# hyunlord/hnm_recommendation

Measured on AMD Instinct MI355X. Metric: recommendations/sec (batched users, K=12) at 1/2/4/8 MI355X; % HBM roofline, higher is better.
Workload: dtype f16+f32; 1 GPU; ncf: BASELINE configs[1] NeuralCF dim=64, full H&M shape, batch=4096 users/rank, K=12; users=1371980, items=105542, batch_per_rank=4096, k=12, parallelism=single, model=NeuralCF, mf_dim=64, weights=init, scan=certified f16 pre-filter + exact fp32 re-scoring (ncf_cert.hip)

## Files before the change

hnm_recommendation_amd/_lib.py:

```python
from __future__ import annotations

import ctypes as C
import os
import threading
import weakref

import torch

PKG = os.path.dirname(os.path.abspath(__file__))
LIB_PATH = os.environ.get("HNM_LIB_PATH") or os.path.join(PKG, "libhnm_mi355x.so")

HNM_OK, HNM_EINVAL, HNM_EOOB, HNM_EHIP, HNM_ENOMEM, HNM_EUNSUPPORTED, HNM_ECOLL = 0, -1, -2, -3, -4, -5, -6

_p = C.c_void_p
_i64 = C.c_int64
_i32 = C.c_int32
_f32 = C.c_float


class NcfWeights(C.Structure):
    _fields_ = [("gmf_user", _p), ("gmf_item", _p), ("mlp_user", _p), ("mlp_item", _p),
                ("w1", _p), ("b1", _p), ("w2", _p), ("b2", _p), ("wp", _p), ("bp", _p),
                ("num_users", _i64), ("num_items", _i64), ("mf", _i32), ("h0", _i32),
                ("h1", _i32), ("h2", _i32), ("item_proj", _p)]
# ... 258 lines not shown
    check(fn("hnm_ctx_enable_timing")(ctx(device), int(on)), "hnm_ctx_enable_timing")


def kernel_timing(device):
    t = C.c_double()
    n = _i64()
    check(fn("hnm_ctx_timing")(ctx(device), C.byref(t), C.byref(n)), "hnm_ctx_timing")
    return t.value, n.value


HNM_OPT_PREFILTER = 1
HNM_OPT_STATS = 3
HNM_OPT_STRIDED = 4
HNM_OPT_DEEP_MFMA = 5
HNM_OPT_LINEAR_MFMA = 6


def set_option(device, option, value):
    idx = _dev_index(device)
    ctx(device)
    with _lock:
        _opts.setdefault(idx, {})[int(option)] = int(value)
    for c in _device_ctxs(idx):
        check(fn("hnm_ctx_set_option")(c.handle, int(option), int(value)), "hnm_ctx_set_option")


def set_prefilter(device, on=True):
    set_option(device, HNM_OPT_PREFILTER, int(bool(on)))


# ... 16 lines not shown
```

hnm_recommendation_amd/csrc/api.hip:

```cpp
#include <stdlib.h>
#include <string.h>

#include "hnm_device.h"
#include "hnm_internal.h"

static thread_local char g_err[512] = "";

void hnm_set_error(const char* fmt, ...) {
  va_list ap;
  va_start(ap, fmt);
  vsnprintf(g_err, sizeof(g_err), fmt, ap);
  va_end(ap);
}

extern "C" int hnm_abi_version(void) { return HNM_ABI_VERSION; }
extern "C" const char* hnm_last_error(void) { return g_err; }

extern "C" hnm_status hnm_ctx_create(int device, hnm_ctx** out) {
  HNM_REQUIRE(out, HNM_EINVAL, "hnm_ctx_create: out is NULL");
  int ndev = 0;
  HNM_HIP_CHECK(hipGetDeviceCount(&ndev));
  HNM_REQUIRE(device >= 0 && device < ndev, HNM_EINVAL, "hnm_ctx_create: no device %d (%d visible)",
              device, ndev);
  const HnmDeviceGuard guard(device);
  hnm_ctx* c = (hnm_ctx*)calloc(1, sizeof(hnm_ctx));
  HNM_REQUIRE(c, HNM_ENOMEM, "hnm_ctx_create: out of host memory");
  c->device = device;
  c->stream = 0;
  hipDeviceProp_t prop;
  if (hipGetDeviceProperties(&prop, device) == hipSuccess) c->num_cus = prop.multiProcessorCount;
  if (c->num_cus <= 0) c->num_cus = 256;
  c->prefilter = 1;
  c->strided = 0;
  c->deep_mfma = 1;
#ifndef HNM_LINEAR_MFMA_DEFAULT
#define HNM_LINEAR_MFMA_DEFAULT 1
#endif
  c->linear_mfma = HNM_LINEAR_MFMA_DEFAULT;
  if (hipMalloc((void**)&c->err_dev, 64) != hipSuccess) {
    free(c);
    hnm_set_error("hnm_ctx_create: hipMalloc of the error word failed");
    return HNM_ENOMEM;
  }
  HNM_HIP_CHECK(hipMemset(c->err_dev, 0, 64));
  HNM_HIP_CHECK(hipEventCreateWithFlags(&c->chain_ev, hipEventDisableTiming));
  HNM_HIP_CHECK(hipStreamCreateWithFlags(&c->side, hipStreamNonBlocking));
  HNM_HIP_CHECK(hipEventCreateWithFlags(&c->side_in, hipEventDisableTiming));
  HNM_HIP_CHECK(hipEventCreateWithFlags(&c->side_out, hipEventDisableTiming));
  c->stats_dev = reinterpret_cast<unsigned long long*>(reinterpret_cast<char*>(c->err_dev) + 8);
  *out = c;
  return HNM_OK;
}

// ... 43 lines not shown
    case HNM_OPT_PREFILTER:
      ctx->prefilter = value != 0;
      return HNM_OK;
    case HNM_OPT_STATS:
      ctx->stats_on = value != 0;
      return HNM_OK;
    case HNM_OPT_STRIDED:
      ctx->strided = value != 0;
      return HNM_OK;
    case HNM_OPT_DEEP_MFMA:
      ctx->deep_mfma = value != 0;
      return HNM_OK;
    case HNM_OPT_LINEAR_MFMA:
      ctx->linear_mfma = value != 0;
      return HNM_OK;
    default:
      hnm_set_error("hnm_ctx_set_option: unknown option %d", option);
      return HNM_EINVAL;
  }
}

extern "C" hnm_status hnm_ctx_prefilter_stats(hnm_ctx* ctx, int64_t* out, int reset) {
  HNM_CTX_DEVICE(ctx);
  return hnm_ctx_prefilter_stats_ex(ctx, out, 3, reset);
}

extern "C" hnm_status hnm_ctx_prefilter_stats_ex(hnm_ctx* ctx, int64_t* out, int n, int reset) {
  HNM_CTX_DEVICE(ctx);
  HNM_REQUIRE(ctx && out, HNM_EINVAL, "ctx/out is NULL");
  HNM_REQUIRE(n >= 1 && n <= HNM_STATS_N, HNM_EINVAL, "prefilter_stats: 1 <= n <= %d", HNM_STATS_N);
// ... 164 lines not shown
extern "C" hnm_status hnm_gather_rows_f32(hnm_ctx* ctx, const float* table, int64_t rows,
                                          int64_t ld, int d, const int64_t* ids, int64_t n,
                                          float* out, int64_t ldo) {
  HNM_CTX_DEVICE(ctx);
  HNM_REQUIRE(ctx && table && ((ids && out) || n == 0), HNM_EINVAL, "gather: NULL argument");
  HNM_REQUIRE(d > 0 && ld >= d && ldo >= d && rows > 0, HNM_EINVAL, "gather: bad shape");
  if (n <= 0) return HNM_OK;
  const bool vec4 = (d % 4 == 0) && (ld % 4 == 0) && (ldo % 4 == 0) &&
                    ((uintptr_t)table % 16 == 0) && ((uintptr_t)out % 16 == 0);
  hipLaunchKernelGGL(gather_rows_kernel, dim3((unsigned)hnm_cdiv(n, 4)), dim3(256), 0,
                     ctx->stream, table, rows, ld, d, ids, n, out, ldo, ctx->err_dev, vec4);
  HNM_LAUNCH_CHECK();
  return HNM_OK;
}

#define LIN_TN 64
#define LIN_TK 32
template <int LIN_TM, bool VEC>
__global__ __launch_bounds__(256) void linear_rows_kernel(
    const float* __restrict__ X, int64_t ldx, const int64_t* __restrict__ ids, int64_t x_rows,
    int64_t M, int K, const float* __restrict__ W, int64_t ldw, const float* __restrict__ bias,
    int N, float* __restrict__ Y, int64_t ldy, int pair_permute, unsigned* err) {
  constexpr int RPT = LIN_TM / 16;
  constexpr int XP = LIN_TM + (VEC ? 4 : 1), WP = LIN_TN + (VEC ? 4 : 1);
  __shared__ __attribute__((aligned(16))) float xs[LIN_TK][XP];
  __shared__ __attribute__((aligned(16))) float ws[LIN_TK][WP];
  const int t = threadIdx.x;
  const int64_t m0 = (int64_t)blockIdx.x * LIN_TM;
  const int n0 = blockIdx.y * LIN_TN;
  const int tr = (t >> 4) * RPT;
  const int tc = (t & 15) * 4;
  float acc[RPT][4] = {};
// ... 84 lines not shown
    for (int j = 0; j < 4; ++j) {
      const int n = n0 + tc + j;
      if (n >= N) continue;
      float v = acc[i][j];
      if (bias) v += bias[n];
      const int64_t c = pair_permute ? (int64_t)(n & 1) * (ldy / 2) + (n >> 1) : n;
      Y[m * ldy + c] = v;
    }
  }
}

__global__ __launch_bounds__(256) void linear_rows_mfma_kernel(
    const float* __restrict__ X, int64_t ldx, const int64_t* __restrict__ ids, int64_t x_rows,
    int64_t M, int K, const float* __restrict__ W, int64_t ldw, const float* __restrict__ bias,
    int N, float* __restrict__ Y, int64_t ldy, int pair_permute, unsigned* err) {
  constexpr int RS = LIN_TK + 1;
  __shared__ float xs[64 * RS];
  __shared__ float ws[64 * RS];
  const int t = threadIdx.x, lane = t & 63, wave = t >> 6;
  const int i = lane & 31, h = lane >> 5;
  const int64_t m0 = (int64_t)blockIdx.x * 64;
  const int n0 = blockIdx.y * LIN_TN;
  const int wr = 32 * (wave >> 1), wc = 32 * (wave & 1);
  f32x16 acc = {};
  for (int k0 = 0; k0 < K; k0 += LIN_TK) {
    for (int e = t; e < 64 * LIN_TK / 4; e += 256) {
      const int rr = e / (LIN_TK / 4), kq = 4 * (e % (LIN_TK / 4));
      const int64_t m = m0 + rr;
      float4 v = make_float4(0.f, 0.f, 0.f, 0.f);
      if (m < M) {
        const int64_t src = ids ? ids[m] : m;
        if (src < 0 || src >= x_rows) {
          if (kq == 0) hnm_flag(err, HNM_ERR_OOB);
          v = make_float4(__builtin_nanf(""), __builtin_nanf(""), __builtin_nanf(""),
                          __builtin_nanf(""));
        } else {
          v = *reinterpret_cast<const float4*>(X + src * ldx + k0 + kq);
        }
      }
      float* xr = xs + rr * RS + kq;
      xr[0] = v.x; xr[1] = v.y; xr[2] = v.z; xr[3] = v.w;
    }
    for (int e = t; e < LIN_TN * LIN_TK / 4; e += 256) {
      const int nn = e / (LIN_TK / 4), kq = 4 * (e % (LIN_TK / 4));
      float4 v = make_float4(0.f, 0.f, 0.f, 0.f);
      if (n0 + nn < N) v = *reinterpret_cast<const float4*>(W + (int64_t)(n0 + nn) * ldw + k0 + kq);
      float* wr4 = ws + nn * RS + kq;
      wr4[0] = v.x; wr4[1] = v.y; wr4[2] = v.z; wr4[3] = v.w;
    }
    __syncthreads();
    const float* xa = xs + (wr + i) * RS + h;
    const float* wb = ws + (wc + i) * RS + h;
#pragma unroll
    for (int st = 0; st < LIN_TK / 2; ++st) acc = mfma32x32x2(xa[2 * st], wb[2 * st], acc);
    __syncthreads();
  }
  const int n = n0 + wc + i;
  if (n >= N) return;
  const float bn = bias ? bias[n] : 0.f;
  const int64_t c = pair_permute ? (int64_t)(n & 1) * (ldy / 2) + (n >> 1) : n;
#pragma unroll
  for (int r = 0; r < 16; ++r) {
    const int64_t m = m0 + wr + mfma32_row(r, h);
    if (m >= M) continue;
    float v = acc[r];
    if (bias) v += bn;
    Y[m * ldy + c] = v;
  }
}

extern "C" hnm_status hnm_linear_rows_f32(hnm_ctx* ctx, const float* X, int64_t ldx,
// ... 436 lines not shown
```

hnm_recommendation_amd/csrc/hnm_internal.h:

```cpp
#pragma once
#include <hip/hip_runtime.h>
#include <stdarg.h>
#include <stdint.h>
#include <stdio.h>

#include <algorithm>

#include "../../include/hnm.h"

struct hnm_ctx {
  int device;
  hipStream_t stream;
  hipEvent_t chain_ev;
  hipStream_t side;
  hipEvent_t side_in, side_out;
  void* ws;
  size_t ws_size;
  unsigned* err_dev;
  int num_cus;
  int timing;
  int nev;
  int cap;
  hipEvent_t* ev0;
  hipEvent_t* ev1;
  int prefilter;
  int strided;
  int deep_mfma;
  int linear_mfma;
  void* comm;
  int comm_owned;
  unsigned long long* stats_dev;
  int stats_on;
  struct {
    int kind;
    int64_t B, I;
    int K;
    const void* ids;
    const void* items;
    int flags;
  } pend;
};
struct HnmDeviceGuard {
  int prev = -1;
// ... 124 lines not shown
```

hnm_recommendation_amd/csrc/ncf.hip:

```cpp
#include <algorithm>

#include "hnm_device.h"
#include "ncf_internal.h"

template <bool DENSE>
__global__ __launch_bounds__(256, 2) void ncf32_kernel(
    const float* __restrict__ Pu,
    const float* __restrict__ WGu,
    const float* __restrict__ Qi,
    const float* __restrict__ Gi, int64_t ldg, int mf,
    const float* __restrict__ W2, int h1, int h2, const float* __restrict__ b2,
    const float* __restrict__ wm, const float* __restrict__ bp, int64_t B, int64_t I,
    int64_t ipp, const int64_t* __restrict__ mptr, const int32_t* __restrict__ midx, int K,
    float* __restrict__ cand_v, int32_t* __restrict__ cand_i, int NP,
    float* __restrict__ dense, int64_t ldo, const int32_t* __restrict__ rows,
    const int32_t* __restrict__ nrows, int dyn_cus) {
  constexpr int KS = 32;
  constexpr int RS = 68;
  constexpr int NU = 128;
  __shared__ __attribute__((aligned(16))) float qs[TILE * RS];
  __shared__ __attribute__((aligned(16))) float gs[TILE * RS];
  __shared__ __attribute__((aligned(16))) float ps[NU * 64];
  __shared__ __attribute__((aligned(16))) float gsm[4 * 32 * 32];
  extern __shared__ __attribute__((aligned(16))) float lists[];
// ... 534 lines not shown
                         const int32_t* nrows, float* cv, int32_t* ci, float* ov, int64_t* oi) {
  const int64_t grid = list_rows_grid(B, w->num_items, ctx->num_cus);
  launch_ncf32<false>(ctx, dim3((unsigned)grid, 1), t, w, B, 0, mptr, midx, K, cv, ci, 1, nullptr,
                      0, rows, nrows, ctx->num_cus);
  HNM_LAUNCH_CHECK();
  return hnm_topk_merge_rows(ctx, cv, ci, B, 1, 0, K, K, K, ov, oi, rows, nrows, w->num_items,
                             ctx->num_cus);
}

struct NcfCall {
  NcfTabs t;
  bool big;
  void* extra;
};

static hnm_status ncf_tables(hnm_ctx* ctx, const hnm_ncf_weights* w, const int64_t* ids,
                             int64_t B, size_t extra, NcfCall* out, bool fill = true) {
  const bool big = w->h1 > 64 || w->mf > 64;
  const int H1P = big ? 128 : 64, GW = big ? 128 : 64;
  const int64_t I = w->num_items;
  const bool gcopy = (big ? w->mf != GW : w->mf % 4 != 0) || ((uintptr_t)w->gmf_item % 16 != 0);
  const bool qcache = w->item_proj != nullptr;
  const size_t szP = hnm_align((size_t)B * H1P * 4), szW = hnm_align((size_t)B * GW * 4);
  const size_t szQ = qcache ? 0 : hnm_align((size_t)I * H1P * 4);
  const size_t szG = gcopy ? hnm_align((size_t)I * GW * 4) : 0;
  void* wsp = ctx->ws;
  hnm_status st = HNM_OK;
  if (fill) {
    st = hnm_workspace(ctx, szP + szW + szQ + szG + extra, &wsp);
    if (st) return st;
  } else {
    HNM_REQUIRE(ctx->ws && ctx->ws_size >= szP + szW + szQ + szG + extra, HNM_EINVAL,
                "ncf: the begin phase's workspace is gone");
  }
  char* base = (char*)wsp;
  float* Pu = (float*)base; base += szP;
  float* WGu = (float*)base; base += szW;
  float* Qi = (float*)base; base += szQ;
  float* Gc = (float*)base; base += szG;
  out->extra = base;
  out->big = big;
  const float* G = w->gmf_item;
  int64_t ldg = w->mf;
  if (gcopy) {
    G = Gc;
    ldg = GW;
  }
  out->t = {Pu, WGu, qcache ? w->item_proj : Qi, G, ldg};
  if (!fill) return HNM_OK;
  if (w->h1 < H1P) {
    HNM_HIP_CHECK(hipMemsetAsync(Pu, 0, szP, ctx->stream));
    if (!qcache) HNM_HIP_CHECK(hipMemsetAsync(Qi, 0, szQ, ctx->stream));
  }
  st = hnm_linear_rows_f32(ctx, w->mlp_user, w->h0, ids, w->num_users, B, w->h0, w->w1,
                           2 * w->h0, w->b1, w->h1, Pu, H1P, 1);
  if (st) return st;
  if (!qcache) {
    st = hnm_linear_rows_f32(ctx, w->mlp_item, w->h0, nullptr, I, I, w->h0, w->w1 + w->h0,
                             2 * w->h0, nullptr, w->h1, Qi, H1P, 1);
    if (st) return st;
  }
  hipLaunchKernelGGL(gather_scale_kernel, dim3((unsigned)hnm_cdiv(B, 4)), dim3(256), 0,
                     ctx->stream, w->gmf_user, w->num_users, w->mf, w->mf, ids, B, w->wp, WGu,
                     GW, ctx->err_dev, big ? 0 : 1);
// ... 13 lines not shown
  hnm_status st = ncf_check(w);
  if (st) return st;
  HNM_REQUIRE(ctx && (ids || B == 0), HNM_EINVAL, "ncf: NULL argument");
  if (B <= 0) return HNM_OK;
  const int64_t I = w->num_items;
  const bool big = w->h1 > 64 || w->mf > 64;
  const bool cert = !DENSE && !big && ctx->prefilter && B >= 16 && ncf_cert_eligible(w, K);
  const int WU = B >= 256 ? 4 : 1;
  const int64_t ublocks = big ? hnm_cdiv(B, 4 * WU) : hnm_cdiv(B, 128);
  const Partition part = choose_partition(I, ublocks, ctx->num_cus);
  const size_t szC = DENSE ? 0 : hnm_align((size_t)B * part.np * K * 4);
  const bool strided = ctx->strided != 0;
  const size_t extra =
      cert ? ncf_cert_bytes(B, I, K, ctx->num_cus, ncf_cert_wg(ctx), strided) : 2 * szC;
  NcfCall c;
  st = ncf_tables(ctx, w, ids, B, extra, &c);
  if (st) return st;
  if (cert) return ncf_cert_topk(ctx, w, c.t, B, mptr, midx, K, c.extra, strided, ov, oi);
  float* cv = (float*)c.extra;
  int32_t* ci = (int32_t*)((char*)c.extra + szC);

  dim3 grid((unsigned)ublocks, (unsigned)part.np);
#define HNM_NCF(WUV)                                                                          \
  if (big)                                                                                    \
    launch_ncf<WUV, 128, 64, DENSE>(ctx, grid, c.t, w, B, part.ipp, mptr, midx, K, cv, ci,    \
                                    part.np, dense, ldo);                                     \
  else                                                                                        \
    launch_ncf<WUV, 64, 32, DENSE>(ctx, grid, c.t, w, B, part.ipp, mptr, midx, K, cv, ci,     \
                                   part.np, dense, ldo);
  hnm_timer_begin(ctx, HNM_TIME_SCORE);
  if (!big) {
// ... 32 lines not shown

static hnm_status ncf_topk_begin(hnm_ctx* ctx, const hnm_ncf_weights* w, const int64_t* user_ids,
                                 int64_t B, const int64_t* mask_ptr, const int32_t* mask_idx,
                                 int k, float* lower_bound, float* lists) {
  hnm_status st = ncf_check(w);
  if (st) return st;
  HNM_REQUIRE(ctx && ((user_ids && (lower_bound || lists)) || B == 0) && k >= 1 && k <= 64,
              HNM_EINVAL, "ncf_topk_begin: bad argument");
  HNM_REQUIRE(!ctx->pend.kind, HNM_EINVAL, "ncf_topk_begin: a two-phase call is already open");
  if (B <= 0) return HNM_OK;
  const bool big = w->h1 > 64 || w->mf > 64;
  const bool cert = !big && ctx->prefilter && ncf_cert_eligible(w, k);
  const bool strided = ctx->strided != 0;
  if (cert) {
    NcfCall c;
    st = ncf_tables(ctx, w, user_ids, B,
                    ncf_cert_bytes(B, w->num_items, k, ctx->num_cus, ncf_cert_wg(ctx), strided),
                    &c);
    if (st) return st;
    st = ncf_cert_begin(ctx, w, c.t, B, mask_ptr, mask_idx, k, c.extra, strided, lower_bound,
                        lists);
    if (st) return st;
  } else {
    if (lower_bound && (st = hnm_fill_f32(ctx, lower_bound, B, -__builtin_inff()))) return st;
    if (lists && (st = hnm_fill_f32(ctx, lists, B * k, -__builtin_inff()))) return st;
  }
  ctx->pend = {cert ? HNM_PEND_NCF_CERT : HNM_PEND_NCF_EXACT, B, w->num_items, k, user_ids,
               w->mlp_item, strided ? HNM_PEND_STRIDED : 0};
  return HNM_OK;
}

extern "C" hnm_status hnm_ncf_topk_begin_f32(hnm_ctx* ctx, const hnm_ncf_weights* w,
                                             const int64_t* user_ids, int64_t B,
// ... 63 lines not shown
}

extern "C" hnm_status hnm_ncf_prefilter_debug_f32(hnm_ctx* ctx, const hnm_ncf_weights* w,
                                                  const int64_t* user_ids, int64_t B,
                                                  float* approx, int64_t lda, float* bound) {
  HNM_CTX_DEVICE(ctx);
  hnm_status st = ncf_check(w);
  if (st) return st;
  HNM_REQUIRE(ctx && user_ids && approx && bound && lda >= w->num_items, HNM_EINVAL,
              "ncf_prefilter_debug: bad argument");
  HNM_REQUIRE(w->h1 <= 64 && w->mf <= 64 && w->num_items * 64 < ((int64_t)1 << 31),
              HNM_EUNSUPPORTED,
              "ncf_prefilter_debug: the f16 pre-filter covers h1 <= 64, mf <= 64, < 2^25 items");
  if (B <= 0) return HNM_OK;
  NcfCall c;
  st = ncf_tables(ctx, w, user_ids, B,
                  ncf_cert_bytes(B, w->num_items, 1, ctx->num_cus, ncf_cert_wg(ctx), false), &c);
  if (st) return st;
  return ncf_cert_debug(ctx, w, c.t, B, c.extra, approx, lda, bound);
}

static void deep_view(const hnm_ncf_deep_weights* dw, const int64_t* ids, hnm_ncf_weights* w,
                      CertDeep* dp) {
  *w = hnm_ncf_weights{};
  w->gmf_user = dw->gmf_user;
  w->gmf_item = dw->gmf_item;
  w->mlp_user = dw->mlp_user;
  w->mlp_item = dw->mlp_item;
  w->w1 = dw->w[0];
  w->b1 = dw->b[0];
  w->w2 = dw->w[1];
  w->b2 = dw->b[1];
// ... 14 lines not shown
      dw->mf % 4 != 0 || (uintptr_t)dw->gmf_item % 16 != 0)
    return false;
  hnm_ncf_weights w;
  CertDeep dp;
  deep_view(dw, nullptr, &w, &dp);
  return ncf_cert_eligible(&w, K);
}

hnm_status ncf_deep_cert(hnm_ctx* ctx, const hnm_ncf_deep_weights* dw, const int64_t* ids,
                         int64_t B, const int64_t* mptr, const int32_t* midx, int K, float* ov,
                         int64_t* oi, int32_t** ovf_rows, int32_t** ovf_cnt, bool* pruned) {
  hnm_ncf_weights w;
  CertDeep dp;
  deep_view(dw, ids, &w, &dp);
  NcfCall c;
  hnm_status st = ncf_tables(
      ctx, &w, ids, B, ncf_cert_bytes(B, w.num_items, K, ctx->num_cus, ncf_cert_wg(ctx), false), &c);
  if (st) return st;
  return ncf_deep_cert_topk(ctx, &w, dp, c.t, B, mptr, midx, K, c.extra, ov, oi, ovf_rows, ovf_cnt,
                            pruned);
}

hnm_status ncf_deep_cert_debug(hnm_ctx* ctx, const hnm_ncf_deep_weights* dw, const int64_t* ids,
                               int64_t B, float* approx, int64_t lda, float* bound) {
  hnm_ncf_weights w;
  CertDeep dp;
  deep_view(dw, ids, &w, &dp);
  NcfCall c;
  hnm_status st = ncf_tables(
      ctx, &w, ids, B, ncf_cert_bytes(B, w.num_items, 1, ctx->num_cus, ncf_cert_wg(ctx), false), &c);
  if (st) return st;
  return ncf_cert_debug(ctx, &w, c.t, B, c.extra, approx, lda, bound, &dp);
}

extern "C" hnm_status hnm_ncf_pair_scores_f32(hnm_ctx* ctx, const hnm_ncf_weights* w,
                                              const int64_t* user_ids, const int64_t* item_ids,
                                              int64_t n, float* out) {
  HNM_CTX_DEVICE(ctx);
  hnm_status st = ncf_check(w);
  if (st) return st;
  HNM_REQUIRE(ctx && ((user_ids && item_ids && out) || n == 0), HNM_EINVAL, "ncf_pair: NULL argument");
  if (n <= 0) return HNM_OK;
  hipLaunchKernelGGL(ncf_pair_kernel, dim3((unsigned)hnm_cdiv(n, 256)), dim3(256), 0, ctx->stream,
                     *w, user_ids, item_ids, n, out, ctx->err_dev);
  HNM_LAUNCH_CHECK();
// ... 3 lines not shown
```

hnm_recommendation_amd/csrc/ncf_cert.hip:

```cpp
#include <algorithm>

#include "hnm_device.h"
#include "ncf_internal.h"
#include "sample_kth.h"

typedef _Float16 h8 __attribute__((ext_vector_type(8)));
typedef _Float16 h4 __attribute__((ext_vector_type(4)));
typedef _Float16 h2 __attribute__((ext_vector_type(2)));


namespace {

constexpr int64_t CERT_MIN_ITEMS = 8192;
constexpr float CERT_RHO = 0.0029296875f;
constexpr float CERT_RHO_DEEP = 0.00390625f;
constexpr int CERT_MAX_NP = 64;
constexpr int CERT_PROXY_USERS = 8;
#ifndef CERT_CHAMPIONS_AB
#define CERT_CHAMPIONS_AB 2048
#endif
constexpr int64_t CERT_CHAMPIONS = CERT_CHAMPIONS_AB;
constexpr int64_t CERT_GROUP_MIN = 48;
constexpr int CERT_STRIDE = 8;
constexpr int64_t CERT_GATE_GAIN = 150;
// ... 1356 lines not shown
    n += bad || !(pd[(int64_t)r * I + i] + 2.f * fmaf(cs, Di[i], Bs[i]) < thr);
#pragma unroll
  for (int o = 32; o >= 1; o >>= 1) n += __shfl_xor(n, o);
  if ((threadIdx.x & 63) == 0 && n) atomicAdd(cnt, (unsigned long long)n);
}

__global__ void cert_unscale_kernel(float* __restrict__ a, float* __restrict__ e, int64_t lda,
                                    int64_t B, int64_t I, const CertParams* __restrict__ prm) {
  const int64_t x = (int64_t)blockIdx.x * 256 + threadIdx.x;
  if (x >= B * I) return;
  const int64_t o = (x / I) * lda + x % I;
  a[o] /= prm->unit;
  e[o] /= prm->unit;
}

struct CertWs {
  CertParams* prm;
  float *Au, *Cu, *Bi, *Di, *tau, *Eu, *b2s, *kthv, *lb, *pdense, *cdense, *part;
  float *Bs, *Cs;
  int32_t* sidx;
  int32_t* sloo;
  int32_t* sidx2;
  float* sdense;
  float* kth2;
  int* gate;
  unsigned long long* gcnt;
  int64_t* kthi;
  int *cnt, *flag;
  int32_t *buf, *ovf_cnt, *ovf_rows;
  float* bufd;
  _Float16 *P16, *WG16, *Q16, *G16, *W2h, *wmh;
  _Float16 *W3h, *wph;
  float *b3s, *u;
  float* cv;
// ... 68 lines not shown
  x.buf = (int32_t*)take((size_t)B * sh.part.np * sh.capp * 4);
  x.bufd = (float*)take((size_t)B * sh.part.np * sh.capp * 4);
  x.P16 = (_Float16*)take((size_t)B * 64 * 2);
  x.WG16 = (_Float16*)take((size_t)B * 64 * 2);
  x.Q16 = (_Float16*)take((size_t)I * 64 * 2);
  x.G16 = (_Float16*)take((size_t)I * 64 * 2);
  x.W2h = (_Float16*)take(32 * 64 * 2);
  x.wmh = (_Float16*)take(32 * 2);
  x.W3h = (_Float16*)take(16 * 32 * 2);
  x.wph = (_Float16*)take(16 * 2);
  x.b3s = (float*)take(16 * 4);
  x.u = (float*)take(32 * 4);
  const size_t lb = ncf_list_bytes(B, I, K, num_cus);
  x.cv = (float*)take(lb);
  x.ci = (int32_t*)take(lb);
  if (w) *w = x;
  return off;
}

hnm_status cert_prepare(hnm_ctx* ctx, const hnm_ncf_weights* w, const NcfTabs& t, int64_t B,
                        const CertWs& x, const CertDeep* dp) {
  const int64_t I = w->num_items;
  const int ib = (int)std::min<int64_t>(1024, hnm_cdiv(I, 4));
  const int ub = (int)std::min<int64_t>(256, hnm_cdiv(B, 4));
  const float* wm = w->wp + w->mf;
  const CertDeep dv = dp ? *dp : CertDeep{};
  if (dp) {
    hipLaunchKernelGGL(cert_deep_u_kernel, dim3(1), dim3(64), 0, ctx->stream, dv, w->h2, x.u);
    HNM_LAUNCH_CHECK();
    wm = x.u;
  }
  hipLaunchKernelGGL(cert_stats_kernel, dim3(ib + ub), dim3(256), 0, ctx->stream, t, B, I, w->mf,
                     w->w2, w->h1, w->h2, wm, x.prm, x.Au, x.Cu, x.Bi, x.Di, x.part, ib, ub);
  HNM_LAUNCH_CHECK();
  hipLaunchKernelGGL(cert_scales_kernel, dim3(1), dim3(256), 0, ctx->stream, w->w2, w->h1, w->h2,
                     w->b2, wm, w->bp, x.prm, x.part, ib, ub, x.ovf_cnt, dv);
  HNM_LAUNCH_CHECK();
  const int cb = (int)std::min<int64_t>(2048, std::max<int64_t>(1, hnm_cdiv(I * 16, 256)));
  hipLaunchKernelGGL(cert_convert_kernel, dim3(cb), dim3(256), 0, ctx->stream, t, B, I, w->mf,
                     x.prm, x.P16, x.WG16, x.Q16, x.G16, w->w2, w->h1, w->h2, w->b2, wm, x.W2h,
                     x.wmh, x.b2s, x.Bi, x.Cu, x.Bs, x.Cs, dv, x.W3h, x.wph, x.b3s);
  HNM_LAUNCH_CHECK();
  return HNM_OK;
}

template <int MODE>
void launch_scan(hnm_ctx* ctx, dim3 grid, const ScanArgs& a) {
  if (a.W3h)
    hipLaunchKernelGGL((ncf16_scan_kernel<MODE, true>), grid, dim3(256), 0, ctx->stream, a);
  else
    hipLaunchKernelGGL((ncf16_scan_kernel<MODE, false>), grid, dim3(256), 0, ctx->stream, a);
// ... 10 lines not shown
  a.G16 = x.G16;
  a.W2h = x.W2h;
  a.wmh = x.wmh;
  a.b2s = x.b2s;
  a.Bi = x.Bs;
  a.Di = x.Di;
  a.Cu = x.Cs;
  a.Eu = x.Eu;
  a.prm = x.prm;
  a.B = B;
  a.sidx = nullptr;
  a.upw = 32;
  return a;
}

}

bool ncf_cert_eligible(const hnm_ncf_weights* w, int K) {
  return w->h1 <= 64 && w->mf <= 64 && w->h2 <= 32 && K <= 64 &&
         w->num_items >= CERT_MIN_ITEMS && w->num_items >= 64 * (int64_t)K &&
         w->num_items * 64 < ((int64_t)1 << 31);
}

int ncf_cert_wg(const hnm_ctx* ctx) {
  (void)ctx;
  return CERT_WG_PER_CU;
}

size_t ncf_cert_bytes(int64_t B, int64_t I, int K, int num_cus, int wg, bool strided) {
  return cert_carve(nullptr, B, I, K, num_cus, wg, strided, nullptr);
// ... 205 lines not shown
```

hnm_recommendation_amd/csrc/ncf_internal.h:

```cpp
#pragma once
#include "hnm_internal.h"

struct NcfTabs {
  const float* Pu;
  const float* WGu;
  const float* Qi;
  const float* G;
  int64_t ldg;
};

hnm_status ncf_list_rows(hnm_ctx* ctx, const hnm_ncf_weights* w, const NcfTabs& t, int64_t B,
                         const int64_t* mptr, const int32_t* midx, int K, const int32_t* rows,
                         const int32_t* nrows, float* cv, int32_t* ci, float* ov, int64_t* oi);
size_t ncf_list_bytes(int64_t B, int64_t I, int K, int num_cus);

struct CertDeep {
  const float* W3;
  const float* b3;
  const float* wp3;
  int h3;
  const float* gmf_user;
  const float* gmf_item;
  const float* wp;
  const int64_t* ids;
};

bool ncf_deep_cert_eligible(const hnm_ncf_deep_weights* dw, int K);
hnm_status ncf_deep_cert(hnm_ctx* ctx, const hnm_ncf_deep_weights* dw, const int64_t* ids,
                         int64_t B, const int64_t* mptr, const int32_t* midx, int K, float* ov,
                         int64_t* oi, int32_t** ovf_rows, int32_t** ovf_cnt, bool* pruned);
hnm_status ncf_deep_cert_debug(hnm_ctx* ctx, const hnm_ncf_deep_weights* dw, const int64_t* ids,
                               int64_t B, float* approx, int64_t lda, float* bound);

bool ncf_cert_eligible(const hnm_ncf_weights* w, int K);
size_t ncf_cert_bytes(int64_t B, int64_t I, int K, int num_cus, int wg, bool strided);
int ncf_cert_wg(const hnm_ctx* ctx);
hnm_status ncf_cert_topk(hnm_ctx* ctx, const hnm_ncf_weights* w, const NcfTabs& t, int64_t B,
                         const int64_t* mptr, const int32_t* midx, int K, void* scratch,
                         bool strided, float* ov, int64_t* oi);
hnm_status ncf_cert_begin(hnm_ctx* ctx, const hnm_ncf_weights* w, const NcfTabs& t, int64_t B,
                          const int64_t* mptr, const int32_t* midx, int K, void* scratch,
                          bool strided, float* lb, float* lists = nullptr,
                          const CertDeep* dp = nullptr);
hnm_status ncf_cert_finish(hnm_ctx* ctx, const hnm_ncf_weights* w, const NcfTabs& t, int64_t B,
                           const int64_t* mptr, const int32_t* midx, int K, void* scratch,
                           bool strided, const float* lb, int short_ok, float* ov, int64_t* oi,
                           const CertDeep* dp = nullptr, int32_t** ovf_rows = nullptr,
                           int32_t** ovf_cnt = nullptr);
hnm_status ncf_deep_cert_topk(hnm_ctx* ctx, const hnm_ncf_weights* w, const CertDeep& dp,
                              const NcfTabs& t, int64_t B, const int64_t* mptr,
                              const int32_t* midx, int K, void* scratch, float* ov, int64_t* oi,
// ... 5 lines not shown
```

include/hnm.h:

```cpp
#ifndef HNM_H_
#define HNM_H_

#include <stddef.h>
#include <stdint.h>

#ifdef __cplusplus
extern "C" {
#endif

#define HNM_ABI_VERSION 1

typedef int32_t hnm_status;
enum {
  HNM_OK = 0,
  HNM_EINVAL = -1,
  HNM_EOOB = -2,
  HNM_EHIP = -3,
  HNM_ENOMEM = -4,
  HNM_EUNSUPPORTED = -5,
  HNM_ECOLL = -6
};

typedef struct hnm_ctx hnm_ctx;
typedef struct hnm_spmm_plan hnm_spmm_plan;

int hnm_abi_version(void);
const char* hnm_last_error(void);

hnm_status hnm_ctx_create(int device, hnm_ctx** out);
hnm_status hnm_ctx_destroy(hnm_ctx* ctx);
hnm_status hnm_ctx_set_stream(hnm_ctx* ctx, void* hip_stream);
hnm_status hnm_ctx_reserve(hnm_ctx* ctx, size_t bytes);
hnm_status hnm_ctx_check(hnm_ctx* ctx);
hnm_status hnm_ctx_num_cus(hnm_ctx* ctx, int* out);
hnm_status hnm_ctx_abort_pending(hnm_ctx* ctx);
enum { HNM_OPT_PREFILTER = 1,
       HNM_OPT_STATS = 3,
       HNM_OPT_STRIDED = 4,
       HNM_OPT_DEEP_MFMA = 5   ,
       HNM_OPT_LINEAR_MFMA = 6  };
hnm_status hnm_ctx_set_option(hnm_ctx* ctx, int option, int64_t value);
hnm_status hnm_ctx_prefilter_stats(hnm_ctx* ctx, int64_t* out, int reset);
hnm_status hnm_ctx_prefilter_stats_ex(hnm_ctx* ctx, int64_t* out, int n, int reset);
hnm_status hnm_ctx_enable_timing(hnm_ctx* ctx, int mask);
hnm_status hnm_ctx_timing(hnm_ctx* ctx, double* total_ms, int64_t* launches);

hnm_status hnm_gather_rows_f32(hnm_ctx* ctx, const float* table, int64_t rows, int64_t ld,
                               int d, const int64_t* ids, int64_t n, float* out,
                               int64_t ldo);

hnm_status hnm_linear_rows_f32(hnm_ctx* ctx, const float* X, int64_t ldx, const int64_t* ids,
                               int64_t x_rows, int64_t M, int K, const float* W,
                               int64_t ldw, const float* bias, int N, float* Y, int64_t ldy,
                               int pair_permute);

// ... 282 lines not shown
```

Measured before the change: 2.010 million users/s.

## Fuse NCF table construction with certification stats into one kernel

Adds a fused kernel that computes the item MLP projection tile (Qi) via MFMA, the user projections (Pu, WGu), and the per-item/per-user certification bounds (Au, Cu, Bi, Di, block maxima) in a single launch. The separate memsets, linear launches and the cert_stats pass, which re-read Qi/Pu from memory, are skipped when the fused path applies. It is on by default for small (h1, mf <= 64) aligned configs, and the shared MFMA tile loop is factored into a header. The risk is lower occupancy or imbalance between the item-block and user-block roles within one grid, and the fused path must reproduce the old stats exactly.

```diff
diff --git a/hnm_recommendation_amd/_lib.py b/hnm_recommendation_amd/_lib.py
--- a/hnm_recommendation_amd/_lib.py
+++ b/hnm_recommendation_amd/_lib.py
@@ -296,6 +296,7 @@
 HNM_OPT_STRIDED = 4
 HNM_OPT_DEEP_MFMA = 5
 HNM_OPT_LINEAR_MFMA = 6
+HNM_OPT_NCF_FUSED = 7
 
 
 def set_option(device, option, value):
diff --git a/hnm_recommendation_amd/csrc/api.hip b/hnm_recommendation_amd/csrc/api.hip
--- a/hnm_recommendation_amd/csrc/api.hip
+++ b/hnm_recommendation_amd/csrc/api.hip
@@ -3,6 +3,7 @@
 
 #include "hnm_device.h"
 #include "hnm_internal.h"
+#include "linear_tile.h"
 
 static thread_local char g_err[512] = "";
 
@@ -37,6 +38,7 @@
 #define HNM_LINEAR_MFMA_DEFAULT 1
 #endif
   c->linear_mfma = HNM_LINEAR_MFMA_DEFAULT;
+  c->ncf_fused = 1;
   if (hipMalloc((void**)&c->err_dev, 64) != hipSuccess) {
     free(c);
     hnm_set_error("hnm_ctx_create: hipMalloc of the error word failed");
@@ -110,6 +112,9 @@
     case HNM_OPT_LINEAR_MFMA:
       ctx->linear_mfma = value != 0;
       return HNM_OK;
+    case HNM_OPT_NCF_FUSED:
+      ctx->ncf_fused = value != 0;
+      return HNM_OK;
     default:
       hnm_set_error("hnm_ctx_set_option: unknown option %d", option);
       return HNM_EINVAL;
@@ -304,8 +309,6 @@
   return HNM_OK;
 }
 
-#define LIN_TN 64
-#define LIN_TK 32
 template <int LIN_TM, bool VEC>
 __global__ __launch_bounds__(256) void linear_rows_kernel(
     const float* __restrict__ X, int64_t ldx, const int64_t* __restrict__ ids, int64_t x_rows,
@@ -420,47 +423,14 @@
     const float* __restrict__ X, int64_t ldx, const int64_t* __restrict__ ids, int64_t x_rows,
     int64_t M, int K, const float* __restrict__ W, int64_t ldw, const float* __restrict__ bias,
     int N, float* __restrict__ Y, int64_t ldy, int pair_permute, unsigned* err) {
-  constexpr int RS = LIN_TK + 1;
-  __shared__ float xs[64 * RS];
-  __shared__ float ws[64 * RS];
-  const int t = threadIdx.x, lane = t & 63, wave = t >> 6;
+  __shared__ float xs[64 * LIN_RS];
+  __shared__ float ws[64 * LIN_RS];
+  const int lane = threadIdx.x & 63, wave = threadIdx.x >> 6;
   const int i = lane & 31, h = lane >> 5;
   const int64_t m0 = (int64_t)blockIdx.x * 64;
   const int n0 = blockIdx.y * LIN_TN;
   const int wr = 32 * (wave >> 1), wc = 32 * (wave & 1);
-  f32x16 acc = {};
-  for (int k0 = 0; k0 < K; k0 += LIN_TK) {
-    for (int e = t; e < 64 * LIN_TK / 4; e += 256) {
-      const int rr = e / (LIN_TK / 4), kq = 4 * (e % (LIN_TK / 4));
-      const int64_t m = m0 + rr;
-      float4 v = make_float4(0.f, 0.f, 0.f, 0.f);
-      if (m < M) {
-        const int64_t src = ids ? ids[m] : m;
-        if (src < 0 || src >= x_rows) {
-          if (kq == 0) hnm_flag(err, HNM_ERR_OOB);
-          v = make_float4(__builtin_nanf(""), __builtin_nanf(""), __builtin_nanf(""),
-                          __builtin_nanf(""));
-        } else {
-          v = *reinterpret_cast<const float4*>(X + src * ldx + k0 + kq);
-        }
-      }
-      float* xr = xs + rr * RS + kq;
-      xr[0] = v.x; xr[1] = v.y; xr[2] = v.z; xr[3] = v.w;
-    }
-    for (int e = t; e < LIN_TN * LIN_TK / 4; e += 256) {
-      const int nn = e / (LIN_TK / 4), kq = 4 * (e % (LIN_TK / 4));
-      float4 v = make_float4(0.f, 0.f, 0.f, 0.f);
-      if (n0 + nn < N) v = *reinterpret_cast<const float4*>(W + (int64_t)(n0 + nn) * ldw + k0 + kq);
-      float* wr4 = ws + nn * RS + kq;
-      wr4[0] = v.x; wr4[1] = v.y; wr4[2] = v.z; wr4[3] = v.w;
-    }
-    __syncthreads();
-    const float* xa = xs + (wr + i) * RS + h;
-    const float* wb = ws + (wc + i) * RS + h;
-#pragma unroll
-    for (int st = 0; st < LIN_TK / 2; ++st) acc = mfma32x32x2(xa[2 * st], wb[2 * st], acc);
-    __syncthreads();
-  }
+  const f32x16 acc = linear_mfma_tile(X, ldx, ids, x_rows, M, K, W, ldw, N, m0, n0, xs, ws, err);
   const int n = n0 + wc + i;
   if (n >= N) return;
   const float bn = bias ? bias[n] : 0.f;
diff --git a/hnm_recommendation_amd/csrc/hnm_internal.h b/hnm_recommendation_amd/csrc/hnm_internal.h
--- a/hnm_recommendation_amd/csrc/hnm_internal.h
+++ b/hnm_recommendation_amd/csrc/hnm_internal.h
@@ -27,6 +27,7 @@
   int strided;
   int deep_mfma;
   int linear_mfma;
+  int ncf_fused;
   void* comm;
   int comm_owned;
   unsigned long long* stats_dev;
diff --git a/hnm_recommendation_amd/csrc/linear_tile.h b/hnm_recommendation_amd/csrc/linear_tile.h
--- /dev/null
+++ b/hnm_recommendation_amd/csrc/linear_tile.h
@@ -0,0 +1,49 @@
+#pragma once
+#include "hnm_device.h"
+
+#define LIN_TN 64
+#define LIN_TK 32
+#define LIN_RS (LIN_TK + 1)
+
+__device__ __forceinline__ f32x16 linear_mfma_tile(
+    const float* __restrict__ X, int64_t ldx, const int64_t* __restrict__ ids, int64_t x_rows,
+    int64_t M, int K, const float* __restrict__ W, int64_t ldw, int N, int64_t m0, int n0,
+    float* xs, float* ws, unsigned* err) {
+  const int t = threadIdx.x, lane = t & 63, wave = t >> 6;
+  const int i = lane & 31, h = lane >> 5;
+  const int wr = 32 * (wave >> 1), wc = 32 * (wave & 1);
+  f32x16 acc = {};
+  for (int k0 = 0; k0 < K; k0 += LIN_TK) {
+    for (int e = t; e < 64 * LIN_TK / 4; e += 256) {
+      const int rr = e / (LIN_TK / 4), kq = 4 * (e % (LIN_TK / 4));
+      const int64_t m = m0 + rr;
+      float4 v = make_float4(0.f, 0.f, 0.f, 0.f);
+      if (m < M) {
+        const int64_t src = ids ? ids[m] : m;
+        if (src < 0 || src >= x_rows) {
+          if (kq == 0) hnm_flag(err, HNM_ERR_OOB);
+          v = make_float4(__builtin_nanf(""), __builtin_nanf(""), __builtin_nanf(""),
+                          __builtin_nanf(""));
+        } else {
+          v = *reinterpret_cast<const float4*>(X + src * ldx + k0 + kq);
+        }
+      }
+      float* xr = xs + rr * LIN_RS + kq;
+      xr[0] = v.x; xr[1] = v.y; xr[2] = v.z; xr[3] = v.w;
+    }
+    for (int e = t; e < LIN_TN * LIN_TK / 4; e += 256) {
+      const int nn = e / (LIN_TK / 4), kq = 4 * (e % (LIN_TK / 4));
+      float4 v = make_float4(0.f, 0.f, 0.f, 0.f);
+      if (n0 + nn < N) v = *reinterpret_cast<const float4*>(W + (int64_t)(n0 + nn) * ldw + k0 + kq);
+      float* wr4 = ws + nn * LIN_RS + kq;
+      wr4[0] = v.x; wr4[1] = v.y; wr4[2] = v.z; wr4[3] = v.w;
+    }
+    __syncthreads();
+    const float* xa = xs + (wr + i) * LIN_RS + h;
+    const float* wb = ws + (wc + i) * LIN_RS + h;
+#pragma unroll
+    for (int st = 0; st < LIN_TK / 2; ++st) acc = mfma32x32x2(xa[2 * st], wb[2 * st], acc);
+    __syncthreads();
+  }
+  return acc;
+}
diff --git a/hnm_recommendation_amd/csrc/ncf.hip b/hnm_recommendation_amd/csrc/ncf.hip
--- a/hnm_recommendation_amd/csrc/ncf.hip
+++ b/hnm_recommendation_amd/csrc/ncf.hip
@@ -572,8 +572,15 @@
   void* extra;
 };
 
+struct NcfFuse {
+  int K;
+  bool strided;
+  const CertDeep* dp;
+};
+
 static hnm_status ncf_tables(hnm_ctx* ctx, const hnm_ncf_weights* w, const int64_t* ids,
-                             int64_t B, size_t extra, NcfCall* out, bool fill = true) {
+                             int64_t B, size_t extra, NcfCall* out, bool fill = true,
+                             const NcfFuse* fuse = nullptr) {
   const bool big = w->h1 > 64 || w->mf > 64;
   const int H1P = big ? 128 : 64, GW = big ? 128 : 64;
   const int64_t I = w->num_items;
@@ -604,8 +611,16 @@
     G = Gc;
     ldg = GW;
   }
-  out->t = {Pu, WGu, qcache ? w->item_proj : Qi, G, ldg};
+  out->t = {Pu, WGu, qcache ? w->item_proj : Qi, G, ldg, 0};
   if (!fill) return HNM_OK;
+  auto al16 = [](const void* p) { return (uintptr_t)p % 16 == 0; };
+  if (fuse && ctx->ncf_fused && !big && !gcopy && !qcache && w->h0 % 32 == 0 &&
+      al16(w->mlp_user) && al16(w->mlp_item) && al16(w->w1)) {
+    st = ncf_cert_fused_tables(ctx, w, ids, B, Pu, WGu, Qi, G, ldg, out->extra, fuse->K,
+                               fuse->strided, fuse->dp);
+    out->t.fused = 1;
+    return st;
+  }
   if (w->h1 < H1P) {
     HNM_HIP_CHECK(hipMemsetAsync(Pu, 0, szP, ctx->stream));
     if (!qcache) HNM_HIP_CHECK(hipMemsetAsync(Qi, 0, szQ, ctx->stream));
@@ -649,7 +664,8 @@
   const size_t extra =
       cert ? ncf_cert_bytes(B, I, K, ctx->num_cus, ncf_cert_wg(ctx), strided) : 2 * szC;
   NcfCall c;
-  st = ncf_tables(ctx, w, ids, B, extra, &c);
+  const NcfFuse fuse{K, strided, nullptr};
+  st = ncf_tables(ctx, w, ids, B, extra, &c, true, cert ? &fuse : nullptr);
   if (st) return st;
   if (cert) return ncf_cert_topk(ctx, w, c.t, B, mptr, midx, K, c.extra, strided, ov, oi);
   float* cv = (float*)c.extra;
@@ -712,9 +728,10 @@
   const bool strided = ctx->strided != 0;
   if (cert) {
     NcfCall c;
+    const NcfFuse fuse{k, strided, nullptr};
     st = ncf_tables(ctx, w, user_ids, B,
                     ncf_cert_bytes(B, w->num_items, k, ctx->num_cus, ncf_cert_wg(ctx), strided),
-                    &c);
+                    &c, true, &fuse);
     if (st) return st;
     st = ncf_cert_begin(ctx, w, c.t, B, mask_ptr, mask_idx, k, c.extra, strided, lower_bound,
                         lists);
@@ -808,8 +825,10 @@
               "ncf_prefilter_debug: the f16 pre-filter covers h1 <= 64, mf <= 64, < 2^25 items");
   if (B <= 0) return HNM_OK;
   NcfCall c;
+  const NcfFuse fuse{1, false, nullptr};
   st = ncf_tables(ctx, w, user_ids, B,
-                  ncf_cert_bytes(B, w->num_items, 1, ctx->num_cus, ncf_cert_wg(ctx), false), &c);
+                  ncf_cert_bytes(B, w->num_items, 1, ctx->num_cus, ncf_cert_wg(ctx), false), &c,
+                  true, &fuse);
   if (st) return st;
   return ncf_cert_debug(ctx, w, c.t, B, c.extra, approx, lda, bound);
 }
@@ -854,8 +873,10 @@
   CertDeep dp;
   deep_view(dw, ids, &w, &dp);
   NcfCall c;
+  const NcfFuse fuse{K, false, &dp};
   hnm_status st = ncf_tables(
-      ctx, &w, ids, B, ncf_cert_bytes(B, w.num_items, K, ctx->num_cus, ncf_cert_wg(ctx), false), &c);
+      ctx, &w, ids, B, ncf_cert_bytes(B, w.num_items, K, ctx->num_cus, ncf_cert_wg(ctx), false), &c,
+      true, &fuse);
   if (st) return st;
   return ncf_deep_cert_topk(ctx, &w, dp, c.t, B, mptr, midx, K, c.extra, ov, oi, ovf_rows, ovf_cnt,
                             pruned);
@@ -867,8 +888,10 @@
   CertDeep dp;
   deep_view(dw, ids, &w, &dp);
   NcfCall c;
+  const NcfFuse fuse{1, false, &dp};
   hnm_status st = ncf_tables(
-      ctx, &w, ids, B, ncf_cert_bytes(B, w.num_items, 1, ctx->num_cus, ncf_cert_wg(ctx), false), &c);
+      ctx, &w, ids, B, ncf_cert_bytes(B, w.num_items, 1, ctx->num_cus, ncf_cert_wg(ctx), false), &c,
+      true, &fuse);
   if (st) return st;
   return ncf_cert_debug(ctx, &w, c.t, B, c.extra, approx, lda, bound, &dp);
 }
diff --git a/hnm_recommendation_amd/csrc/ncf_cert.hip b/hnm_recommendation_amd/csrc/ncf_cert.hip
--- a/hnm_recommendation_amd/csrc/ncf_cert.hip
+++ b/hnm_recommendation_amd/csrc/ncf_cert.hip
@@ -1,6 +1,7 @@
 #include <algorithm>
 
 #include "hnm_device.h"
+#include "linear_tile.h"
 #include "ncf_internal.h"
 #include "sample_kth.h"
 
@@ -1394,10 +1395,254 @@
   e[o] /= prm->unit;
 }
 
+
+__device__ __forceinline__ void stats_vt(const float* __restrict__ W2, int h1, int h2,
+                                         const float* __restrict__ wm, float* vs) {
+  const int tid = threadIdx.x;
+  if (tid < 64) {
+    float v = 0.f;
+    const int k = korig(tid);
+    if (k < h1) {
+      float w2[32];
+#pragma unroll
+      for (int j = 0; j < 32; ++j) w2[j] = W2[std::min(j, h2 - 1) * h1 + k];
+#pragma unroll
+      for (int j = 0; j < 32; ++j)
+        if (j < h2) v += fabsf(wm[j]) * fabsf(w2[j]);
+    }
+    vs[tid] = v;
+  }
+  __syncthreads();
+}
+
+__device__ __forceinline__ void stats_items4(float vt, const float (&aq)[4], const float (&g)[4],
+                                             int64_t i0, int64_t stride, int64_t I, int lane,
+                                             float* __restrict__ Bi, float* __restrict__ Di,
+                                             float& m0, float& m1, float& m2, float& m3) {
+  float v8[8];
+#pragma unroll
+  for (int u = 0; u < 4; ++u) {
+    v8[u] = vt * aq[u];
+    v8[4 + u] = g[u] * g[u];
+    if (i0 + u * stride < I) {
+      m0 = nmax(m0, aq[u]);
+      m1 = nmax(m1, fabsf(g[u]));
+    }
+  }
+  const bool b5 = lane & 32, b4 = lane & 16, b3 = lane & 8;
+  float w4[4], w2[2];
+#pragma unroll
+  for (int q = 0; q < 4; ++q)
+    w4[q] = (b5 ? v8[2 * q + 1] : v8[2 * q]) + __shfl_xor(b5 ? v8[2 * q] : v8[2 * q + 1], 32);
+#pragma unroll
+  for (int q = 0; q < 2; ++q)
+    w2[q] = (b4 ? w4[2 * q + 1] : w4[2 * q]) + __shfl_xor(b4 ? w4[2 * q] : w4[2 * q + 1], 16);
+  float w1 = (b3 ? w2[1] : w2[0]) + __shfl_xor(b3 ? w2[0] : w2[1], 8);
+  w1 += __shfl_xor(w1, 4);
+  w1 += __shfl_xor(w1, 2);
+  w1 += __shfl_xor(w1, 1);
+  const int idx = (b5 ? 1 : 0) + (b4 ? 2 : 0) + (b3 ? 4 : 0);
+  const int64_t i = i0 + (idx & 3) * stride;
+  if (i < I) {
+    if (idx < 4) {
+      m2 = nmax(m2, w1);
+      if ((lane & 7) == 0) Bi[i] = w1;
+    } else {
+      const float dq = sqrtf(w1);
+      m3 = nmax(m3, dq);
+      if ((lane & 7) == 0) Di[i] = dq;
+    }
+  }
+}
+
+__device__ __forceinline__ void stats_user(float vt, float pu, float wg, int64_t b, int lane,
+                                           float* __restrict__ Au, float* __restrict__ Cu,
+                                           float& m0, float& m1) {
+  const float ap = fabsf(pu);
+  m0 = nmax(m0, ap);
+  m1 = nmax(m1, fabsf(wg));
+  const float a = wave_sum(vt * ap), c2 = wave_sum(wg * wg);
+  if (lane == 0) {
+    Au[b] = a;
+    Cu[b] = sqrtf(c2);
+  }
+}
+
+__device__ __forceinline__ void stats_block_max(float m0, float m1, float m2, float m3,
+                                                float (*red)[4], float* __restrict__ part,
+                                                int slot) {
+  const int tid = threadIdx.x, lane = tid & 63, wave = tid >> 6;
+  m0 = wave_max(m0);
+  m1 = wave_max(m1);
+  m2 = wave_max(m2);
+  m3 = wave_max(m3);
+  if (lane == 0) {
+    red[wave][0] = m0;
+    red[wave][1] = m1;
+    red[wave][2] = m2;
+    red[wave][3] = m3;
+  }
+  __syncthreads();
+  if (tid < 4) {
+    float m = red[0][tid];
+    for (int w = 1; w < 4; ++w) m = nmax(m, red[w][tid]);
+    part[slot * 4 + tid] = m;
+  }
+}
+
+struct TabStatArgs {
+  const float* Xi;
+  const float* Xu;
+  const float* Gu;
+  const int64_t* ids;
+  int64_t num_users, B, I;
+  int h0, h1, h2, mf;
+  const float* W1;
+  const float* b1;
+  const float* wp;
+  const float* W2;
+  const float* wm;
+  float* Pu;
+  float* WGu;
+  float* Qi;
+  const float* G;
+  int64_t ldg;
+  float *Au, *Cu, *Bi, *Di, *part;
+  int item_blocks, user_blocks;
+  unsigned* err;
+};
+
+constexpr int TS_QRS = 65;
+constexpr int TS_UPB = 16;
+
+__global__ __launch_bounds__(256) void ncf_tables_stats_kernel(TabStatArgs a) {
+  __shared__ __attribute__((aligned(16))) float sm[2 * 64 * LIN_RS];
+  __shared__ float vs[64];
+  __shared__ float red[4][4];
+  static_assert(64 * TS_QRS <= 2 * 64 * LIN_RS && (LIN_TK + TS_UPB) * 64 <= 2 * 64 * LIN_RS,
+                "the finished tile and the user step reuse the operand buffers");
+  const int tid = threadIdx.x, lane = tid & 63, wave = tid >> 6;
+  stats_vt(a.W2, a.h1, a.h2, a.wm, vs);
+  const float vt = vs[lane];
+  float m0 = 0.f, m1 = 0.f, m2 = 0.f, m3 = 0.f;
+  const int ib = (int)blockIdx.x - a.user_blocks;
+  const int slot = ib >= 0 ? ib : a.item_blocks + (int)blockIdx.x;
+  if (ib >= 0) {
+    const int i = lane & 31, h = lane >> 5;
+    const int wr = 32 * (wave >> 1), n = 32 * (wave & 1) + i;
+    const int c = (n & 1) * 32 + (n >> 1);
+    const int64_t ntiles = hnm_cdiv(a.I, 64);
+    for (int64_t tile = ib; tile < ntiles; tile += a.item_blocks) {
+      const int64_t r0 = tile * 64;
+      float gv[16];
+#pragma unroll
+      for (int r = 0; r < 16; ++r) {
+        const int64_t it = std::min<int64_t>(r0 + wave * 16 + r, a.I - 1);
+        gv[r] = lane < a.mf ? a.G[it * a.ldg + lane] : 0.f;
+      }
+      const f32x16 acc = linear_mfma_tile(a.Xi, a.h0, nullptr, a.I, a.I, a.h0, a.W1 + a.h0,
+                                          2 * (int64_t)a.h0, a.h1, r0, 0, sm, sm + 64 * LIN_RS,
+                                          a.err);
+#pragma unroll
+      for (int r = 0; r < 16; ++r)
+        sm[(wr + mfma32_row(r, h)) * TS_QRS + c] = n < a.h1 ? acc[r] : 0.f;
+      __syncthreads();
+#pragma unroll
+      for (int s = 0; s < 4; ++s) {
+        const int row = wave * 16 + 4 * s;
+        const int64_t i0 = r0 + row;
+        if (i0 >= a.I) break;
+        float aq[4], g[4];
+#pragma unroll
+        for (int u = 0; u < 4; ++u) {
+          const int64_t it = i0 + u;
+          const float q = sm[(row + u) * TS_QRS + lane];
+          if (it < a.I) a.Qi[it * 64 + lane] = q;
+          aq[u] = fabsf(q);
+          g[u] = gv[4 * s + u];
+        }
+        stats_items4(vt, aq, g, i0, 1, a.I, lane, a.Bi, a.Di, m0, m1, m2, m3);
+      }
+      __syncthreads();
+    }
+  } else {
+    float* wsT = sm;
+    float* xs = sm + LIN_TK * 64;
+    const int nout = korig(lane);
+    const int ub = (int)blockIdx.x;
+    for (int64_t b0 = (int64_t)ub * TS_UPB; b0 < a.B; b0 += (int64_t)a.user_blocks * TS_UPB) {
+      float acc[4] = {0.f, 0.f, 0.f, 0.f};
+      for (int k0 = 0; k0 < a.h0; k0 += LIN_TK) {
+        for (int e = tid; e < 64 * LIN_TK / 4; e += 256) {
+          const int t = e / (LIN_TK / 4), kq = 4 * (e % (LIN_TK / 4));
+          const int o = korig(t);
+          float4 v = make_float4(0.f, 0.f, 0.f, 0.f);
+          if (o < a.h1) v = *reinterpret_cast<const float4*>(a.W1 + (int64_t)o * 2 * a.h0 + k0 + kq);
+          wsT[(kq + 0) * 64 + t] = v.x;
+          wsT[(kq + 1) * 64 + t] = v.y;
+          wsT[(kq + 2) * 64 + t] = v.z;
+          wsT[(kq + 3) * 64 + t] = v.w;
+        }
+        if (tid < TS_UPB * LIN_TK / 4) {
+          const int rr = tid / (LIN_TK / 4), kq = 4 * (tid % (LIN_TK / 4));
+          const int64_t b = b0 + rr;
+          float4 v = make_float4(0.f, 0.f, 0.f, 0.f);
+          if (b < a.B) {
+            const int64_t src = a.ids[b];
+            if (src < 0 || src >= a.num_users) {
+              if (kq == 0 && k0 == 0) hnm_flag(a.err, HNM_ERR_OOB);
+              v = make_float4(__builtin_nanf(""), __builtin_nanf(""), __builtin_nanf(""),
+                              __builtin_nanf(""));
+            } else {
+              v = *reinterpret_cast<const float4*>(a.Xu + src * a.h0 + k0 + kq);
+            }
+          }
+          *reinterpret_cast<float4*>(xs + rr * LIN_TK + kq) = v;
+        }
+        __syncthreads();
+#pragma unroll 8
+        for (int kk = 0; kk < LIN_TK; ++kk) {
+          const float wv = wsT[kk * 64 + lane];
+#pragma unroll
+          for (int u = 0; u < 4; ++u) acc[u] = fmaf(xs[(4 * wave + u) * LIN_TK + kk], wv, acc[u]);
+        }
+        __syncthreads();
+      }
+      const float bn = nout < a.h1 ? a.b1[nout] : 0.f;
+#pragma unroll
+      for (int u = 0; u < 4; ++u) {
+        const int64_t b = b0 + 4 * wave + u;
+        if (b >= a.B) break;
+        const float pu = nout < a.h1 ? acc[u] + bn : 0.f;
+        const int64_t id = a.ids[b];
+        const bool ok = id >= 0 && id < a.num_users;
+        const float wg = (ok && nout < a.mf) ? a.Gu[id * a.mf + nout] * a.wp[nout] : 0.f;
+        a.Pu[b * 64 + lane] = pu;
+        a.WGu[b * 64 + lane] = wg;
+        stats_user(vt, pu, wg, b, lane, a.Au, a.Cu, m0, m1);
+      }
+    }
+  }
+  stats_block_max(m0, m1, m2, m3, red, a.part, slot);
+}
+
+constexpr int STATS_MAX_IB = 2048;
+void stats_grid(int64_t I, int64_t B, bool fused, int* ib, int* ub) {
+  if (fused) {
+    const int64_t ntiles = hnm_cdiv(I, 64), per = hnm_cdiv(ntiles, STATS_MAX_IB);
+    *ib = (int)hnm_cdiv(ntiles, per);
+    *ub = (int)std::min<int64_t>(256, hnm_cdiv(B, TS_UPB));
+  } else {
+    *ib = (int)std::min<int64_t>(1024, hnm_cdiv(I, 4));
+    *ub = (int)std::min<int64_t>(256, hnm_cdiv(B, 4));
+  }
+}
+
 struct CertWs {
   CertParams* prm;
   float *Au, *Cu, *Bi, *Di, *tau, *Eu, *b2s, *kthv, *lb, *pdense, *cdense, *part;
   float *Bs, *Cs;
+  float* partf;
   int32_t* sidx;
   int32_t* sloo;
   int32_t* sidx2;
@@ -1496,6 +1741,7 @@
   const size_t lb = ncf_list_bytes(B, I, K, num_cus);
   x.cv = (float*)take(lb);
   x.ci = (int32_t*)take(lb);
+  x.partf = (float*)take(4 * 4 * (STATS_MAX_IB + 256));
   if (w) *w = x;
   return off;
 }
@@ -1503,20 +1749,22 @@
 hnm_status cert_prepare(hnm_ctx* ctx, const hnm_ncf_weights* w, const NcfTabs& t, int64_t B,
                         const CertWs& x, const CertDeep* dp) {
   const int64_t I = w->num_items;
-  const int ib = (int)std::min<int64_t>(1024, hnm_cdiv(I, 4));
-  const int ub = (int)std::min<int64_t>(256, hnm_cdiv(B, 4));
-  const float* wm = w->wp + w->mf;
+  int ib, ub;
+  stats_grid(I, B, t.fused != 0, &ib, &ub);
+  const float* wm = dp ? x.u : w->wp + w->mf;
   const CertDeep dv = dp ? *dp : CertDeep{};
-  if (dp) {
-    hipLaunchKernelGGL(cert_deep_u_kernel, dim3(1), dim3(64), 0, ctx->stream, dv, w->h2, x.u);
+  const float* part = t.fused ? x.partf : x.part;
+  if (!t.fused) {
+    if (dp) {
+      hipLaunchKernelGGL(cert_deep_u_kernel, dim3(1), dim3(64), 0, ctx->stream, dv, w->h2, x.u);
+      HNM_LAUNCH_CHECK();
+    }
+    hipLaunchKernelGGL(cert_stats_kernel, dim3(ib + ub), dim3(256), 0, ctx->stream, t, B, I, w->mf,
+                       w->w2, w->h1, w->h2, wm, x.prm, x.Au, x.Cu, x.Bi, x.Di, x.part, ib, ub);
     HNM_LAUNCH_CHECK();
-    wm = x.u;
-  }
-  hipLaunchKernelGGL(cert_stats_kernel, dim3(ib + ub), dim3(256), 0, ctx->stream, t, B, I, w->mf,
-                     w->w2, w->h1, w->h2, wm, x.prm, x.Au, x.Cu, x.Bi, x.Di, x.part, ib, ub);
-  HNM_LAUNCH_CHECK();
+  }
   hipLaunchKernelGGL(cert_scales_kernel, dim3(1), dim3(256), 0, ctx->stream, w->w2, w->h1, w->h2,
-                     w->b2, wm, w->bp, x.prm, x.part, ib, ub, x.ovf_cnt, dv);
+                     w->b2, wm, w->bp, x.prm, part, ib, ub, x.ovf_cnt, dv);
   HNM_LAUNCH_CHECK();
   const int cb = (int)std::min<int64_t>(2048, std::max<int64_t>(1, hnm_cdiv(I * 16, 256)));
   hipLaunchKernelGGL(cert_convert_kernel, dim3(cb), dim3(256), 0, ctx->stream, t, B, I, w->mf,
@@ -1557,6 +1805,54 @@
   return a;
 }
 
+}
+
+hnm_status ncf_cert_fused_tables(hnm_ctx* ctx, const hnm_ncf_weights* w, const int64_t* ids,
+                                 int64_t B, float* Pu, float* WGu, float* Qi, const float* G,
+                                 int64_t ldg, void* scratch, int K, bool strided,
+                                 const CertDeep* dp) {
+  const int64_t I = w->num_items;
+  CertWs x;
+  cert_carve((char*)scratch, B, I, K, ctx->num_cus, ncf_cert_wg(ctx), strided, &x);
+  const float* wm = w->wp + w->mf;
+  if (dp) {
+    hipLaunchKernelGGL(cert_deep_u_kernel, dim3(1), dim3(64), 0, ctx->stream, *dp, w->h2, x.u);
+    HNM_LAUNCH_CHECK();
+    wm = x.u;
+  }
+  TabStatArgs a{};
+  a.Xi = w->mlp_item;
+  a.Xu = w->mlp_user;
+  a.Gu = w->gmf_user;
+  a.ids = ids;
+  a.num_users = w->num_users;
+  a.B = B;
+  a.I = I;
+  a.h0 = w->h0;
+  a.h1 = w->h1;
+  a.h2 = w->h2;
+  a.mf = w->mf;
+  a.W1 = w->w1;
+  a.b1 = w->b1;
+  a.wp = w->wp;
+  a.W2 = w->w2;
+  a.wm = wm;
+  a.Pu = Pu;
+  a.WGu = WGu;
+  a.Qi = Qi;
+  a.G = G;
+  a.ldg = ldg;
+  a.Au = x.Au;
+  a.Cu = x.Cu;
+  a.Bi = x.Bi;
+  a.Di = x.Di;
+  a.part = x.partf;
+  stats_grid(I, B, true, &a.item_blocks, &a.user_blocks);
+  a.err = ctx->err_dev;
+  hipLaunchKernelGGL(ncf_tables_stats_kernel, dim3(a.item_blocks + a.user_blocks), dim3(256), 0,
+                     ctx->stream, a);
+  HNM_LAUNCH_CHECK();
+  return HNM_OK;
 }
 
 bool ncf_cert_eligible(const hnm_ncf_weights* w, int K) {
diff --git a/hnm_recommendation_amd/csrc/ncf_internal.h b/hnm_recommendation_amd/csrc/ncf_internal.h
--- a/hnm_recommendation_amd/csrc/ncf_internal.h
+++ b/hnm_recommendation_amd/csrc/ncf_internal.h
@@ -7,6 +7,7 @@
   const float* Qi;
   const float* G;
   int64_t ldg;
+  int fused;
 };
 
 hnm_status ncf_list_rows(hnm_ctx* ctx, const hnm_ncf_weights* w, const NcfTabs& t, int64_t B,
@@ -35,6 +36,10 @@
 bool ncf_cert_eligible(const hnm_ncf_weights* w, int K);
 size_t ncf_cert_bytes(int64_t B, int64_t I, int K, int num_cus, int wg, bool strided);
 int ncf_cert_wg(const hnm_ctx* ctx);
+hnm_status ncf_cert_fused_tables(hnm_ctx* ctx, const hnm_ncf_weights* w, const int64_t* ids,
+                                 int64_t B, float* Pu, float* WGu, float* Qi, const float* G,
+                                 int64_t ldg, void* scratch, int K, bool strided,
+                                 const CertDeep* dp);
 hnm_status ncf_cert_topk(hnm_ctx* ctx, const hnm_ncf_weights* w, const NcfTabs& t, int64_t B,
                          const int64_t* mptr, const int32_t* midx, int K, void* scratch,
                          bool strided, float* ov, int64_t* oi);
diff --git a/include/hnm.h b/include/hnm.h
--- a/include/hnm.h
+++ b/include/hnm.h
@@ -38,7 +38,8 @@
        HNM_OPT_STATS = 3,
        HNM_OPT_STRIDED = 4,
        HNM_OPT_DEEP_MFMA = 5   ,
-       HNM_OPT_LINEAR_MFMA = 6  };
+       HNM_OPT_LINEAR_MFMA = 6 ,
+       HNM_OPT_NCF_FUSED = 7    };
 hnm_status hnm_ctx_set_option(hnm_ctx* ctx, int option, int64_t value);
 hnm_status hnm_ctx_prefilter_stats(hnm_ctx* ctx, int64_t* out, int reset);
 hnm_status hnm_ctx_prefilter_stats_ex(hnm_ctx* ctx, int64_t* out, int n, int reset);
```

Result: no change. 2.011 million users/s, median of 2 (+0.0%).
